# menickname/waafle

Hardware: AMD Instinct MI355X
Metric: contigs scored/sec + k2 clade-pair evals/sec at 1/2/4/8 MI355X vs CPU ref (higher is better)
Workload: dtype f64

## Files before the change

waafle_amd/csrc/wf_device.h:

```cpp
#pragma once
#include "wf_internal.h"

#include "waafle_hip.h"
#include "wf_lanes.h"

namespace wf {

namespace {


constexpr uint64_t kKeyPad = ~0ull;

#include "wf_stamps.h"
constexpr int kLocVirtual = 0xFFFF;

__device__ __forceinline__ void note_ppot(const KArgs& K, int c, int iteration, int Pp) {
  if (!K.ppot || Pp < 2) return;
  const uint64_t old = (uint64_t)K.ppot[c];
  if (iteration > (int)(old >> 40))
    K.ppot[c] = (int64_t)(((uint64_t)iteration << 40) | ((old & ((1ull << 40) - 1ull)) + (uint64_t)Pp));
}

__device__ __forceinline__ bool e2_no_option(const KArgs& K, int c, int iteration, int64_t pair_evals, bool root,
                                             int32_t* pend) {
// ... 309 lines not shown
    a7 = a6; a6 = a5; a5 = a4; a4 = a3; a3 = a2; a2 = a1; a1 = a0; a0 = v;
    pop();
    --sp;
    while (sp > 0) {
      if (ss[0] == 1) {
        int h = sl[0] / 2;
        h -= h % 8;
        ss[0] = 2;
        push(so[0] + h, sl[0] - h);
        ++sp;
        break;
      }
      a0 = a1 + a0;
      a1 = a2; a2 = a3; a3 = a4; a4 = a5; a5 = a6; a6 = a7;
      pop();
      --sp;
    }
  }
  return a0;
}

template <class F>
__device__ __forceinline__ double np_sum(int n, F f) {
  if (n <= kLeafMax) return 0.0 + serial_block(0, n, f);
  double total = 0.0;
  for (int o = 0; o < n; o += kNpyBuf) total += serial_pairwise(o, min(kNpyBuf, n - o), f);
  return total;
}


struct Contig {
  int64_t h0, l0, mbase;
  int H, G;
  int *loc_lo, *loc_len, *loc_st, *leaf_off;
  int *loc_grp, *loc_steps, *sched_off;
  uint64_t* sched;
  int4* leaves;
  int *alo, *ahi, *ahit, *aloc, *acl;
  double* asc;
  uint64_t* maxes;
  int *ign, *um;
  uint64_t* keys;
  int *seg_start, *seg_cl, *cl_id, *pot, *mem1, *mem2, *sorder;
  double* S;
  uint64_t* mask;
  unsigned *bm1, *bm2;
  uint8_t* best_syn;
  char* xws = nullptr;
  int64_t xcap = 0;
  int* sib_of = nullptr;
  uint64_t* hm = nullptr;
};

struct SumStack {
  double s0 = 0.0, s1 = 0.0, s2 = 0.0, s3 = 0.0, s4 = 0.0, s5 = 0.0, s6 = 0.0, s7 = 0.0;
  __device__ __forceinline__ void push(double v) {
    s7 = s6; s6 = s5; s5 = s4; s4 = s3; s3 = s2; s2 = s1; s1 = s0; s0 = v;
  }
  __device__ __forceinline__ void add_top() {
    s0 = s1 + s0;
    s1 = s2; s2 = s3; s3 = s4; s4 = s5; s5 = s6; s6 = s7;
  }
};

__device__ __forceinline__ double seqsum(double v, int cnt) {
  double r = 0.0;
  for (int i = 0; i < cnt; ++i) r += v;
  return r;
}

__device__ __forceinline__ double leaf_tree(double r0, double r1, double r2, double r3, double r4,
                                            double r5, double r6, double r7) {
  return ((r0 + r1) + (r2 + r3)) + ((r4 + r5) + (r6 + r7));
}

__device__ __forceinline__ int below(int base, int bound, int m) {
  const int d = bound - base;
  return d <= 0 ? 0 : min(m, (d + 7) >> 3);
}

constexpr int kThreadLeaves = 32;
constexpr int kE2Seg = 320;
constexpr int kE2MaxG = 63;
constexpr int kPruneMax = 64;

constexpr double kEnvSlack = 2e-12;
template <class Rg, class Sc>
__device__ __forceinline__ double env_integral(Rg range, Sc score, int kb, int ke, int len, double& best) {
  double acc = 0.0;
  best = 0.0;
  for (int p = 0; p < len;) {
    int nx = len;
    double val = 0.0;
    for (int q = kb; q < ke; ++q) {
      int l, h;
      range(q, l, h);
      if (l >= h) continue;
      if (l <= p && p < h) {
        const double s = score(q);
        val = s > val ? s : val;
        nx = h < nx ? h : nx;
      } else if (l > p) {
        nx = l < nx ? l : nx;
      }
    }
    best = val > best ? val : best;
    acc += val * (double)(nx - p);
    p = nx;
  }
  return acc / (double)len;
}
__device__ __forceinline__ double marker_ub(double v) { return -1.0 - v; }
__device__ __forceinline__ double marker_lb(double v) {
  const double ub = -1.0 - v;
  const double lb = ub * (1.0 - 5e-12) - 4.5e-16 * (1.0 + ub);
  return lb > 0.0 ? lb : 0.0;
}

__device__ __forceinline__ bool attaches(const DevParams& P, int qlo, int qhi, int hs, int l1,
                                         int len, int lst) {
  if (P.stranded && hs != lst) return false;
  const int l2 = l1 + len - 1;
  if (l1 > qhi || qlo > l2) return 0.0 >= P.min_overlap;
  const int ov = min(qhi, l2) - max(qlo, l1) + 1;
  const int den = min(qhi - qlo + 1, l2 - l1 + 1);
  if (ov == den) return 1.0 >= P.min_overlap;
  const double t = (double)den * P.min_overlap;
  if ((double)ov > t + fabs(t) * 1e-9) return true;
  if ((double)ov < t - fabs(t) * 1e-9) return false;
  return (double)ov / (double)den >= P.min_overlap;
}

__device__ __forceinline__ double run_leaf(int lo, int hi, double v, int st, int ln) {
  const int m = ln >> 3, be = st + (m << 3);
  hi = max(hi, lo);
  double res = 0.0;
  if (m > 0) {
    int k[8], kmin = m;
#pragma unroll
    for (int c = 0; c < 8; ++c) {
      k[c] = below(st + c, hi, m) - below(st + c, lo, m);
      kmin = min(kmin, k[c]);
    }
    double s0 = 0.0;
    for (int i = 0; i < kmin; ++i) s0 += v;
    const double s1 = s0 + v, s2 = s1 + v;
    double r[8];
#pragma unroll
    for (int c = 0; c < 8; ++c) r[c] = k[c] == kmin ? s0 : (k[c] == kmin + 1 ? s1 : s2);
    res = leaf_tree(r[0], r[1], r[2], r[3], r[4], r[5], r[6], r[7]);
  }
  for (int x = be; x < st + ln; ++x) res += (x >= lo && x < hi) ? v : 0.0;
  return res;
}

template <class F>
__device__ __forceinline__ double np_sum_seq(int n, F next) {
  if (n < 8) {
    double r = 0.0;
    for (int i = 0; i < n; ++i) r += next();
    return r;
  }
  double r0 = next(), r1 = next(), r2 = next(), r3 = next();
  double r4 = next(), r5 = next(), r6 = next(), r7 = next();
  int i = 8;
  const int m = n - (n & 7);
// ... 1339 lines not shown
```

waafle_amd/csrc/wf_sparse.h:

```cpp
constexpr int kSpCls = 128;
constexpr int kSpPairs = 128;
constexpr int kSpMemG = 2048;
constexpr int kSpParG = 4096;
constexpr int kSpDense = 16384;
constexpr int kSpWin = 256;
constexpr int kSpMaxG = 63;
constexpr int kSpP1 = 8;

struct SpMember {
  int rs, cl, pi, sp;
  int h, pad;
  unsigned long long hm;
};
struct SpParent {
  unsigned long long key, c1, c2, c3;
};
constexpr int kSpLPar = 64;
static_assert(kSpLPar * 32 == kSpCls * (8 + 4 + 4), "lpar overlays the class table");
constexpr int64_t kSpOffGidx = (int64_t)kSpMemG * sizeof(SpMember);
constexpr int64_t kSpOffPar = kSpOffGidx + (int64_t)kSpMemG * sizeof(int);
constexpr int64_t kSpOffDense = kSpOffPar + (int64_t)kSpParG * sizeof(SpParent);
constexpr int64_t kSpOffUrow = kSpOffDense + (int64_t)kSpDense * sizeof(double);
constexpr int64_t kSpOffBm = kSpOffUrow + 64 * sizeof(double);
constexpr int64_t kSpSlot = kSpOffBm + 2 * (kSpMemG / 32) * sizeof(unsigned);
// ... 800 lines not shown
      lca1 = a1;
      lca2v = a2;
      bool keepit = true;
      if (!P.allow_lca) {
        const int nl = lca2(K, lca1, lca2v);
        keepit = !(nl == lca1 || nl == lca2v);
      }
      have_ok = keepit;
    } else if (kind == 1) {
      have_ok = __shfl(best_ok, 0, 64) != 0;
    } else if (kind == 3) {
      have_ok = true;
    }
    if (have_ok) {
      if (lane < G) K.syn[l0 + lane] = sh.syn[lane];
      if (kind == 2) {
        int o1 = 0, o2 = 0;
        for (int base = 0; base < M; base += 64) {
          const int q = base + lane;
          const bool in1 = in_bm(bm1, q), in2 = in_bm(bm2, q);
          const uint64_t w1 = __ballot(in1), w2 = __ballot(in2);
          if (in1) K.meld[mbase + o1 + __popcll(w1 & below)] = mem[q].cl;
          if (in2) K.meld[mbase + m1 + o2 + __popcll(w2 & below)] = mem[q].cl;
          o1 += __popcll(w1);
          o2 += __popcll(w2);
        }
      }
      if (lane == 0) {
        K.call[c] = WF_CALL_LGT;
        K.crit[c] = best_crit;
        K.rank[c] = pr;
        K.dir[c] = (int8_t)best_dir;
        K.c1[c] = (kind == 2) ? lca1 : mem[best_c1].cl;
        K.c2[c] = (kind == 2) ? lca2v : mem[best_c2].cl;
        K.nm1[c] = (kind == 2) ? m1 : 0;
        K.nm2[c] = (kind == 2) ? m2 : 0;
        K.iters[c] = (int16_t)iteration;
        K.pair_evals[c] = pair_evals;
      }
      BLAP(9);
      return true;
    }
  }
  const int dec = (no_rows || root_present) ? kDecStop : kDecRaise;
  if (dec == kDecRaise && iteration + 1 <= kMaxIter) {
    if (S.seed_pend) {
      if (lane == 0) {
        S.seed_pend[c] = 2;
        K.pair_evals[c] = pair_evals;
      }
      return true;
    }
    sp_raise(S, c, pair_evals);
    BLAP(9);
    return true;
  }
  if (lane == 0) {
    const int it = dec == kDecRaise ? iteration + 1 : iteration;
    K.iters[c] = (int16_t)min(it, 32767);
    K.pair_evals[c] = pair_evals;
    K.status[c] = dec == kDecRaise ? WF_E_RUNAWAY : 0;
  }
  return true;
}

struct E2Shared {
  union {
    struct {
      int2 cg[kE2Seg];
      unsigned long long pm[64];
    };
    unsigned short cand[64 * 63 / 2];
  };
  double v[kE2Seg];
  int t[64], cl[64], par[64], sibp[64];
  unsigned long long pres[64], hm[64], s1[64], s2[64];
  int len[64];
};

__device__ __forceinline__ double e2_at(const E2Shared& sh, int t, uint64_t pres, int g) {
  return ((pres >> g) & 1ull) ? sh.v[t + __popcll(pres & ((1ull << g) - 1ull))] : 0.0;
}

__device__ __forceinline__ double e2_rank(const E2Shared& sh, int a, int b, uint64_t um, int Gu) {
  const int ta = sh.t[a], tb = sh.t[b];
  const uint64_t pa = sh.pres[a], pb = sh.pres[b];
  uint64_t m = um;
  auto next = [&]() -> double {
    const int g = __builtin_ctzll(m);
    m &= m - 1;
    const double x = e2_at(sh, ta, pa, g), y = e2_at(sh, tb, pb, g);
    return x < y ? y : x;
  };
  return (0.0 + np_sum_seq(Gu, next)) / (double)Gu;
}

struct E2Eval {
  int ok, swapped, dir;
  uint64_t mm, mA, mB;
};

__device__ __forceinline__ E2Eval e2_eval(const KArgs& K, const E2Shared& sh, int a, int b, uint64_t um) {
  const DevParams& P = K.p;
  const bool unk = sh.cl[a] == K.unknown || sh.cl[b] == K.unknown;
  uint64_t mm = 0, ma = 0, mb = 0;
  {
    const int ta = sh.t[a], tb = sh.t[b];
    const uint64_t pa = sh.pres[a], pb = sh.pres[b];
    for (uint64_t r = um; r; r &= r - 1) {
      const int g = __builtin_ctzll(r);
      const uint64_t bit = 1ull << g;
      const double s1 = e2_at(sh, ta, pa, g), s2 = e2_at(sh, tb, pb, g);
      const double mn = s2 < s1 ? s2 : s1;
      if (mn >= P.k_amb && !unk) mm |= bit;
      else if (s1 >= P.k2) ma |= bit;
      else if (s2 >= P.k2) mb |= bit;
    }
  }
  E2Eval e;
  const uint64_t ab = ma | mb;
  e.swapped = (ab && ((mb >> __builtin_ctzll(ab)) & 1ull)) ? 1 : 0;
  e.mm = mm;
  e.mA = e.swapped ? mb : ma;
  e.mB = e.swapped ? ma : mb;
  int64_t tot = 0, amb = 0;
  int state = 0;
  bool dir_ok = true;
  for (uint64_t r = um; r; r &= r - 1) {
    const int g = __builtin_ctzll(r);
    const uint64_t bit = 1ull << g;
    const char c = (mm & bit) ? '*' : (e.mA & bit) ? 'A' : (e.mB & bit) ? 'B' : '!';
    if (c != '!') {
      tot += sh.len[g];
      if (c == '*') amb += sh.len[g];
    }
    if (state == 0) { if (c == 'A') state = 1; else dir_ok = false; }
    else if (state == 1) { if (c == 'B') state = 2; else if (c != 'A') dir_ok = false; }
    else if (state == 2) { if (c == 'A') state = 3; else if (c != 'B') dir_ok = false; }
    else { if (c != 'A') dir_ok = false; }
  }
  e.dir = (dir_ok && state == 3) ? 1 : 0;
  e.ok = 1;
  if ((double)amb / (double)tot > P.amb_frac) e.ok = 0;
  if (P.clade_genes >= 0 && min(__popcll(e.mA), __popcll(e.mB)) < P.clade_genes) e.ok = 0;
  const int x = e.swapped ? b : a, y = e.swapped ? a : b;
  if (P.clade_leaves >= 0) {
    const int64_t ly = K.leaves[sh.cl[y]];
    const int64_t lc = e.dir ? ly : min(K.leaves[sh.cl[x]], ly);
    if (lc < P.clade_leaves) e.ok = 0;
  }
  if (P.sister_on && e.ok) {
    const int px = sh.par[x], py = sh.par[y];
    const uint64_t fb = sh.sibp[y] == px ? (sh.s2[x] | (sh.s1[x] & ~sh.hm[y])) : sh.s1[x];
    uint64_t fa = 0;
    if (!e.dir) fa = sh.sibp[x] == py ? (sh.s2[y] | (sh.s1[y] & ~sh.hm[x])) : sh.s1[y];
    if ((fb & e.mB) || (fa & e.mA)) e.ok = 0;
  }
  return e;
}

__device__ __forceinline__ int e2_wave_lca(const KArgs& K, int acc) {
#pragma unroll
  for (int off = 32; off > 0; off >>= 1) acc = lca2(K, acc, __shfl_xor(acc, off, 64));
  return acc;
}

__device__ __forceinline__ bool sp_two(const SArgs& S, E2Shared& sh, int c, int so, int se, uint64_t hdr,
                                       int64_t h0, int64_t l0, int G, int level) {
  const KArgs& K = S.k;
  const DevParams& P = K.p;
  const int lane = threadIdx.x & 63;
  const uint64_t below = (1ull << lane) - 1ull;
  const int ns = se - so;
  if (G > kE2MaxG || ns > kE2Seg) return false;
  SLAP_MARK(c);
  SSTAT(8, 1);
  SSTAT(9, ns);
  const uint64_t um = hdr & ~(1ull << 63);
  const bool root = (hdr >> 63) != 0ull;
  const int Gu = __popcll(um);
  const uint64_t allG = (1ull << G) - 1ull;
  const int iteration = level + 1;
  int64_t pair_evals = level == 0 ? 0 : K.pair_evals[c];
  constexpr int kCh = kE2Seg / 64;
  {
    int2 cgr[kCh];
    double vr[kCh];
#pragma unroll
    for (int k = 0; k < kCh; ++k) {
      const int q = 64 * k + lane;
      cgr[k] = make_int2(-1, 0);
      vr[k] = 0.0;
      if (q < ns) {
        cgr[k] = S.dump_cg[so + q];
        vr[k] = S.dump_mean[so + q];
      }
    }
    int ln = 0;
    if (lane < G) {
      const int ls = K.lstart[l0 + lane], le = K.lend[l0 + lane];
      ln = max(ls, le) - min(ls, le) + 1;
    }
#pragma unroll
    for (int k = 0; k < kCh; ++k) {
      const int q = 64 * k + lane;
      if (q < ns) {
        sh.cg[q] = cgr[k];
        sh.v[q] = vr[k];
      }
    }
    if (lane < G) sh.len[lane] = ln;
  }
  __syncthreads();
  SLAP(0);
  int Pp = 0;
  int hcl[kCh];
  uint64_t hh[kCh];
#pragma unroll
  for (int k = 0; k < kCh; ++k) {
    const int t = 64 * k + lane;
    bool pot = false;
    uint64_t pres = 0, mk2 = 0, hm = 0;
    int cl = -1;
    if (t < ns) {
      cl = sh.cg[t].x;
      if (t == 0 || sh.cg[t - 1].x != cl) {
        for (int q = t; q < ns && sh.cg[q].x == cl; ++q) {
          const uint64_t bit = 1ull << sh.cg[q].y;
          const double x = sh.v[q];
          pres |= bit;
          if (x >= P.k2) mk2 |= bit;
          if (x >= P.sister_thr) hm |= bit;
        }
        const uint64_t miss = allG & ~pres;
        if (0.0 >= P.k2) mk2 |= miss;
        if (0.0 >= P.sister_thr) hm |= miss;
        pot = mk2 != 0ull;
      } else {
        cl = -1;
      }
    }
    hcl[k] = cl;
    hh[k] = hm;
    const uint64_t pb = __ballot(pot);
    const int i = Pp + __popcll(pb & below);
    if (pot && i < 64) {
      sh.t[i] = t; sh.cl[i] = cl;
      sh.pres[i] = pres; sh.pm[i] = mk2 & um; sh.hm[i] = hm; sh.s1[i] = 0; sh.s2[i] = 0;
    }
    Pp += __popcll(pb);
  }
  if (Pp > 64) return false;
  __syncthreads();
  SLAP(1);
  SSTAT(10, Pp);
  const uint64_t my_pm = lane < Pp ? sh.pm[lane] : 0ull;
  pair_evals += (int64_t)Pp * (Pp - 1) / 2;
  if (lane == 0) note_ppot(K, c, iteration, Pp);
  __syncthreads();
  int nc = 0;
  const int n_pairs = Pp * (Pp - 1) / 2;
  for (int p0 = 0; p0 < n_pairs; p0 += 64) {
    const int p = min(p0 + lane, n_pairs - 1);
    int j = (int)((1.0f + __fsqrt_rn(1.0f + 8.0f * (float)p)) * 0.5f);
    j -= j * (j - 1) / 2 > p ? 1 : 0;
    j += (j + 1) * j / 2 <= p ? 1 : 0;
    const int i = p - j * (j - 1) / 2;
    const uint64_t mi = (uint64_t)__shfl((long long)my_pm, i, 64), mj = (uint64_t)__shfl((long long)my_pm, j, 64);
    const bool cand = p0 + lane < n_pairs && (mi | mj) == um;
    const uint64_t cb = __ballot(cand);
    if (cand) sh.cand[nc + __popcll(cb & below)] = (unsigned short)(i | (j << 8));
    nc += __popcll(cb);
  }
  __syncthreads();
  uint64_t memb = 0;
  for (int q = lane; q < nc; q += 64) memb |= (1ull << (sh.cand[q] & 0xFF)) | (1ull << (sh.cand[q] >> 8));
#pragma unroll
  for (int off = 32; off > 0; off >>= 1) memb |= (uint64_t)__shfl_xor((long long)memb, off, 64);
  SLAP(2);
  SSTAT(11, nc);
  if (P.sister_on && memb) {
    const bool me = (memb >> lane) & 1ull;
    const int my_cl = me ? sh.cl[lane] : -1;
    const int my_par = me ? K.parent[my_cl] : -2;
    if (me) {
      sh.par[lane] = my_par;
      sh.sibp[lane] = K.sibp[my_cl];
    }
    int hsp[kCh];
#pragma unroll
    for (int k = 0; k < kCh; ++k) hsp[k] = (hcl[k] >= 0 && hh[k] != 0ull) ? K.sibp[hcl[k]] : -1;
    uint64_t s1 = 0, s2 = 0;
#pragma unroll
    for (int k = 0; k < kCh; ++k) {
      if (64 * k >= ns) break;
      const int sp = hsp[k], cl = hcl[k];
      const uint64_t h = hh[k];
      bool match = false;
      for (uint64_t r = memb; r; r &= r - 1) match = match || (sp >= 0 && sp == lane_bcast(my_par, __builtin_ctzll(r)));
      for (uint64_t mb = __ballot(match); mb; mb &= mb - 1) {
        const int src = __builtin_ctzll(mb);
        const int sp_r = lane_bcast(sp, src), cl_r = lane_bcast(cl, src);
        const uint64_t h_r = lane_bcast(h, src);
        if (my_par == sp_r && my_cl != cl_r) {
          s2 |= s1 & h_r;
          s1 |= h_r;
        }
      }
    }
    if (me) { sh.s1[lane] = s1; sh.s2[lane] = s2; }
    __syncthreads();
  }
  SLAP(3);
  double pr = -__builtin_inf();
  long long pk = -1;
  if (nc > 0) {
    for (int q = lane; q < nc; q += 64) {
      const int i = sh.cand[q] & 0xFF, j = sh.cand[q] >> 8;
      const double r = e2_rank(sh, i, j, um, Gu);
      const long long key = (long long)i * Pp + j;
      if (better(r, key, pr, pk)) { pr = r; pk = key; }
    }
    each_stride([&](auto J) {
      constexpr int js = decltype(J)::value;
      const double r2 = xor_lanes<js>(pr);
      const long long k2 = xor_lanes<js>(pk);
      if (better(r2, k2, pr, pk)) { pr = r2; pk = k2; }
    });
  }
  SLAP(4);
  if (pk >= 0) {
    const int bi = (int)(pk / Pp), bj = (int)(pk % Pp);
    const E2Eval be = e2_eval(K, sh, bi, bj, um);
    int n_in = 0;
    bool all_ok = true, all_same = true;
    uint64_t b1 = 0, b2 = 0;
    for (int q = lane; q < nc; q += 64) {
      const int i = sh.cand[q] & 0xFF, j = sh.cand[q] >> 8;
      if ((pr - e2_rank(sh, i, j, um, Gu)) <= P.range) {
        const E2Eval e = e2_eval(K, sh, i, j, um);
        ++n_in;
        all_ok = all_ok && e.ok;
        all_same = all_same && e.mm == be.mm && e.mA == be.mA && e.mB == be.mB;
        b1 |= 1ull << (e.swapped ? j : i);
        b2 |= 1ull << (e.swapped ? i : j);
      }
    }
#pragma unroll
    for (int off = 32; off > 0; off >>= 1) {
      n_in += __shfl_xor(n_in, off, 64);
      b1 |= (uint64_t)__shfl_xor((long long)b1, off, 64);
      b2 |= (uint64_t)__shfl_xor((long long)b2, off, 64);
    }
    all_ok = __ballot(!all_ok) == 0ull;
    all_same = __ballot(!all_same) == 0ull;
    int kind;
    if (n_in == 0) kind = (P.dis2 == 0) ? 3 : (P.dis2 == 1 ? 0 : 4);
    else if (n_in == 1 || P.dis2 == 0) kind = 1;
    else if (P.dis2 == 1) kind = 0;
    else kind = (all_ok && all_same) ? 2 : 0;
    if (kind == 4) {
      if (lane == 0) K.status[c] = WF_E_BADINPUT;
      return true;
    }
    bool have_ok = false;
    int lca1 = -1, lca2v = -1;
    const bool in1 = (b1 >> lane) & 1ull, in2 = (b2 >> lane) & 1ull;
    const int my_cl = lane < Pp ? sh.cl[lane] : -1;
    if (kind == 2) {
      lca1 = e2_wave_lca(K, in1 ? my_cl : -1);
      lca2v = e2_wave_lca(K, in2 ? my_cl : -1);
      bool keep = true;
      if (!P.allow_lca) {
        const int nl = lca2(K, lca1, lca2v);
        keep = !(nl == lca1 || nl == lca2v);
      }
      have_ok = keep;
    } else if (kind == 1) {
      have_ok = be.ok != 0;
    } else if (kind == 3) {
      have_ok = true;
    }
    if (have_ok) {
      const int64_t mbase = 2 * h0 + 2 * (int64_t)c;
      const int m1 = __popcll(b1), m2 = __popcll(b2);
      if (kind == 2) {
        if (in1) K.meld[mbase + __popcll(b1 & below)] = my_cl;
        if (in2) K.meld[mbase + m1 + __popcll(b2 & below)] = my_cl;
      }
      if (lane < G) {
        const uint64_t bit = 1ull << lane;
        K.syn[l0 + lane] = !(um & bit) ? '~' : (be.mm & bit) ? '*' : (be.mA & bit) ? 'A' : (be.mB & bit) ? 'B' : '!';
      }
      if (lane == 0) {
        double bcrit = 0.0;
        bool first = true;
        const int ta = sh.t[bi], tb = sh.t[bj];
        const uint64_t pa = sh.pres[bi], pb = sh.pres[bj];
        for (uint64_t r = um; r; r &= r - 1) {
          const int g = __builtin_ctzll(r);
          const double x = e2_at(sh, ta, pa, g), y = e2_at(sh, tb, pb, g);
          const double m = x < y ? y : x;
          bcrit = (first || m < bcrit) ? m : bcrit;
          first = false;
        }
        K.call[c] = WF_CALL_LGT;
        K.crit[c] = bcrit;
        K.rank[c] = pr;
        K.dir[c] = (int8_t)be.dir;
        K.c1[c] = kind == 2 ? lca1 : sh.cl[be.swapped ? bj : bi];
        K.c2[c] = kind == 2 ? lca2v : sh.cl[be.swapped ? bi : bj];
        K.nm1[c] = kind == 2 ? m1 : 0;
        K.nm2[c] = kind == 2 ? m2 : 0;
        K.iters[c] = (int16_t)iteration;
        K.pair_evals[c] = pair_evals;
      }
      SLAP(5);
      return true;
    }
  }
  SLAP(5);
  e2_no_option(K, c, iteration, pair_evals, root, S.seed_pend);
  return true;
}

__global__ __launch_bounds__(64, 4) void k_big_sparse(const SArgs S_arg, int level, int64_t n_keys) {
  __shared__ SpShared sh;
  char* ws = S_arg.sp_ws + (int64_t)blockIdx.x * kSpSlot;
  const int count = (int)S_arg.counters[2];
  for (int i = blockIdx.x; i < count; i += gridDim.x) {
    const SArgs& S = kernarg_fresh<SArgs>(S_arg);
    const int cr = S.big_list[2 * i], c = S.big_list[2 * i + 1];
    const bool ok = sp_level(S, sh, ws, c, cr, level, n_keys);
    if (!ok && threadIdx.x == 0) {
      const int slot = (int)atomicAdd(&S.counters[1], 1ull);
      S.big2_list[2 * slot] = cr;
      S.big2_list[2 * slot + 1] = c;
    }
    __syncthreads();
  }
}

template <int KIND>
__global__ __launch_bounds__(64, KIND ? 4 : 2) void k_dump_sparse(const SArgs S_arg, int64_t* ccnt, int64_t* cleaves,
                                                                  int level) {
  using Sh = typename std::conditional<KIND == 1, E2Shared, SpShared>::type;
  __shared__ Sh sh;
  const int lane = threadIdx.x & 63;
  const SArgs& S0 = S_arg;
  if (KIND == 1) {
    if (S0.dump_ctr_next && blockIdx.x == 0 && lane == 0) *S0.dump_ctr_next = 0ull;
    if (S0.anc) {
      const int up = level == 0 ? S0.k.p.jump + 1 : 1;
      for (int t = blockIdx.x * 64 + lane; t < S0.n_tax; t += gridDim.x * 64) {
        int x = level == 0 ? t : S0.anc[t];
        for (int j = 0; j < up; ++j) x = S0.k.parent[x];
        S0.anc[t] = x;
      }
    }
  }
  char* ws = KIND ? nullptr : S0.sp_ws + (int64_t)blockIdx.x * kSpSlot;
  const int count = (int)(*S0.dump_ctr >> 40);
  const int stride = (int)gridDim.x;
  auto finish = [&](const SArgs& S, int c, bool ok) {
    if (lane == 0) {
      const int pd = S.seed_pend[c];
      if (!ok) {
        S.seed_pend[c] = 1;
        if (S.fail_ctr) atomicAdd(S.fail_ctr, 1ull);
      } else if (pd == 3) {
        S.seed_pend[c] = 0;
        ccnt[c] = 0;
        cleaves[c] = 0;
      } else if (pd == 2 && S.roll_next) {
        S.roll_next[atomicAdd(S.roll_next_n, 1ull)] = c;
      }
    }
    __syncthreads();
  };
  for (int base = blockIdx.x; base < count; base += 64 * stride) {
    const int my = base + lane * stride;
    int mc = -1, so = 0, se = 0, G = 0;
    uint64_t hdr = 0;
    int64_t h0 = 0, l0 = 0;
    if (my < count) {
      const int2 dl = reinterpret_cast<const int2*>(S0.dump_list)[my];
      if (dl.x == KIND && dl.y >= 0) {
        mc = dl.y;
        if (KIND == 1) {
          so = S0.dump_first[my];
// ... 25 lines not shown
```

waafle_amd/csrc/wf_staged.hip:

```cpp
#include <hipcub/hipcub.hpp>

#include <algorithm>
#include <atomic>
#include <cstdlib>
#include <string>
#include <vector>

#include "wf_attach.h"

namespace wf {

namespace {

__device__ __forceinline__ int upper_index(const int64_t* off, int n, int64_t x) {
  int lo = 0, hi = n - 1;
  while (lo < hi) {
    const int mid = (lo + hi + 1) >> 1;
    if (off[mid] <= x) lo = mid; else hi = mid - 1;
  }
  return lo;
}

__device__ __forceinline__ int lower_bound_i32(const int32_t* a, int n, int x) {
  int lo = 0, hi = n;
// ... 1438 lines not shown
        cl[r] = a < a1 ? S.att_clade[a] : 0;
      }
#pragma unroll
      for (int r = 0; r < 4; ++r) cl[r] = K.parent[cl[r]];
#pragma unroll
      for (int r = 0; r < 4; ++r) {
        const int64_t a = ab + r * NT + tid;
        if (a < a1) S.att_clade[a] = cl[r];
      }
    }
    STAMP_SYNC();
    STAMP(19);
    return true;
  }
  if (tid == 0) {
    const int it = dec == kDecRaise ? iteration + 1 : iteration;
    K.iters[c] = (int16_t)min(it, 32767);
    K.pair_evals[c] = pair_evals;
    K.status[c] = dec == kDecRaise ? WF_E_RUNAWAY : ctl.status;
  }
  return true;
}

constexpr int kDecNT = 64;

template <int PHASE, int NT = kDecNT>
__global__ __launch_bounds__(NT, 2) void k_decide(const SArgs S, int n_act,
                                                   int level, int64_t n_keys) {
  lvl_counts(S, n_act, n_keys);
  extern __shared__ __attribute__((aligned(16))) char smem[];
  __shared__ Ctl ctl;
  if constexpr (PHASE == 3) {
    const int c1 = (int)S.counters[6], c2 = (int)S.counters[5];
    for (int i = blockIdx.x; i < c1 + c2; i += gridDim.x) {
      const bool whole = i < c1;
      const int32_t* L = whole ? S.one_list : S.two_list;
      const int j = whole ? i : i - c1;
      const int cr = L[2 * j], c = L[2 * j + 1];
      const bool ok = whole ? decide_contig<NT, 0>(S, c, cr, level, smem, S.dec_lds_bytes, ctl, n_keys)
                            : decide_contig<NT, 2>(S, c, cr, level, smem, S.dec_lds_bytes, ctl, n_keys);
      if (!ok && threadIdx.x == 0) {
        const int slot = (int)atomicAdd(&S.counters[2], 1ull);
        S.big_list[2 * slot] = cr;
        S.big_list[2 * slot + 1] = c;
        atomicMax(&S.counters[3], (unsigned long long)S.k.need[c]);
      }
      __syncthreads();
    }
  } else {
  const int32_t* list = PHASE == 1 ? S.one_list : S.two_list;
  const int count = PHASE == 1 ? (list ? (int)S.counters[6] : n_act) : (int)S.counters[5];
  for (int i = blockIdx.x; i < count; i += gridDim.x) {
    const int cr = list ? list[2 * i] : i;
    const int c = list ? list[2 * i + 1] : (S.act ? S.act[cr] : cr);
    const bool ok = decide_contig<NT, PHASE>(S, c, cr, level, smem, S.dec_lds_bytes, ctl, n_keys);
    if (!ok && threadIdx.x == 0) {
      const int slot = (int)atomicAdd(&S.counters[2], 1ull);
      S.big_list[2 * slot] = cr;
      S.big_list[2 * slot + 1] = c;
      atomicMax(&S.counters[3], (unsigned long long)S.k.need[c]);
    }
    __syncthreads();
  }
  }
}

__global__ __launch_bounds__(kBlock, 2) void k_decide_big(const SArgs S, int level,
                                                          int64_t n_keys, int use2) {
  int n_act_ = 0;
  lvl_counts(S, n_act_, n_keys);
  const int count = (int)S.counters[use2 ? 1 : 2];
  const int32_t* list = use2 ? S.big2_list : S.big_list;
  __shared__ Ctl ctl;
  char* base = S.k.big_ws + (int64_t)blockIdx.x * S.k.slot_bytes;
  for (int i = blockIdx.x; i < count; i += gridDim.x) {
    const int cr = list[2 * i], c = list[2 * i + 1];
    const bool ok = decide_contig<kBlock, 0>(S, c, cr, level, base, S.k.slot_bytes, ctl, n_keys, false);
    if (!ok && threadIdx.x == 0) S.k.status[c] = WF_E_NOMEM;
    __syncthreads();
  }
}

#include "wf_sparse.h"
WF_STAMP_READER(sparse, g_sstamps, 16)
WF_STAMP_READER(big, g_bstamps, 48)

int bits_for(int64_t v) {
  int b = 1;
  while (b < 62 && (int64_t(1) << b) <= v) ++b;
  return b;
}

struct Buf {
  void* p = nullptr;
  size_t n = 0;
  ~Buf() { if (p) (void)hipFree(p); }
  hipError_t ensure(hipStream_t drain, size_t bytes) {
    if (bytes <= n) return hipSuccess;
    if (p) {
      hipError_t e = hipStreamSynchronize(drain);
      if (e != hipSuccess) return e;
      (void)hipFree(p);
      p = nullptr;
      n = 0;
    }
    size_t want = std::max<size_t>(bytes + bytes / 4, 256);
    hipError_t e = hipMalloc(&p, want);
    if (e == hipSuccess) n = want;
    return e;
  }
  template <class T> T* as() const { return static_cast<T*>(p); }
};

}



struct StagedState {
  int device = 0;
  int cus = 256;
  Buf lut_off, lut, cnt, att_off, counters, pinned_dummy;
  Buf att_lo, att_hi, att_loc, att_clade, att_hit, att_sc;
  Buf keys0, keys1, vals0, vals1, flags, seg_id, seg_start, seg_crank, seg_mean;
  Buf cnt_leaves, red, seg_nleaf, leaf_off, leaf_seg, leaf_val, annot_best;
  Buf seg_rec, seg_cg, crank_first, satt_lohi, satt_sc, wave_list, lvl_ctr, seg_cnt, seg_len;
  Buf front;
  Buf span_cnt, spans;
  unsigned long long* host_lvl = nullptr;
  hipEvent_t lvl_ev[2] = {nullptr, nullptr};
  int sparse_big = 3;
  int sparse_res = -1;
  int two_res = -1;
  int64_t att_limit = (int64_t(1) << 31) - 1;
  int64_t dump_cap = 0;
  int triage = 1;
  int wave_two = 2;
  Buf tri_list, tri_cnt;
  Buf wq;
  Buf roll0, roll1, roll_cnt, anc;
  bool timing = false;
  std::vector<hipEvent_t> tev;
  int tev_used = 0;
  std::vector<int> tspans;
  double phase_ms[8] = {0};
  int64_t phase_n[8] = {0};
  Buf act0, act1, base0, base1, big_list, big2_list, two_list, one_list, big_ws, tmp, pend, act_l0;
  Buf sp_ws;
  Buf hkey;
  Buf dump_cg, dump_mean, dump_first, dump_list, dump_ctr, dump_um;
  bool level0 = true;
  bool rollup = false;
  bool lut_ready = false;
  int64_t dec_lds = 32 * 1024;
  bool dec_lds_fixed = false;
  unsigned long long* host_counters = nullptr;
  unsigned long long* mbox = nullptr;
  unsigned long long* mbox_dev = nullptr;
  unsigned long long mbox_seq = 0;
  ~StagedState() {
    for (hipEvent_t e : tev) (void)hipEventDestroy(e);
    if (mbox) (void)hipHostFree(mbox);
    if (host_counters) (void)hipHostFree(host_counters);
    if (host_lvl) (void)hipHostFree(host_lvl);
    for (hipEvent_t e : lvl_ev)
      if (e) (void)hipEventDestroy(e);
  }
};
// ... 863 lines not shown
```

waafle_amd/csrc/wf_stamps.h:

```cpp
#pragma once
#ifdef WF_STAMPS
#ifndef WF_STAMPS_ROLL
#define WF_STAMPS_ROLL 0
#endif
#define WF_STAMPS_ONLY(...) __VA_ARGS__
#define WF_STAMP_READER(tag, arr, n)                                                          \
  extern "C" int wf_stamps_read_##tag(unsigned long long* out, int m) {                       \
    if (m > (n)) m = (n);                                                                     \
    return hipMemcpyFromSymbol(out, HIP_SYMBOL(arr), sizeof(unsigned long long) * m) == hipSuccess ? 0 : -2; \
  }                                                                                           \
  extern "C" int wf_stamps_reset_##tag(void) {                                                \
    unsigned long long z[n] = {0};                                                            \
    return hipMemcpyToSymbol(HIP_SYMBOL(arr), z, sizeof z) == hipSuccess ? 0 : -2;            \
  }
__device__ unsigned long long g_stamps[32];
__shared__ unsigned long long g_tlast;
#define STAMP_INIT() do { if (threadIdx.x == 0) g_tlast = __builtin_amdgcn_s_memtime(); } while (0)
#define STAMP(i)                                                                    \
  do {                                                                              \
    if (threadIdx.x == 0) {                                                         \
      unsigned long long now_ = __builtin_amdgcn_s_memtime();                       \
      atomicAdd(&g_stamps[i], now_ - g_tlast);                                      \
      g_tlast = now_;                                                               \
    }                                                                               \
  } while (0)
#define STAMP_SYNC() __syncthreads()
#define LAP_MARK() unsigned long long lap_ = __builtin_amdgcn_s_memtime()
#define LAP(i)                                                                      \
  do {                                                                              \
    unsigned long long n_ = __builtin_amdgcn_s_memtime();                           \
    if (threadIdx.x == 0) atomicAdd(&g_stamps[i], n_ - lap_);                       \
    lap_ = n_;                                                                      \
  } while (0)
#define LAP_WAIT_LDS() __builtin_amdgcn_s_waitcnt(0xc07f)
#define LAP_WAIT_V(v) asm volatile("" ::"v"(v))
#define STAT(i, v) do { if (threadIdx.x == 0) atomicAdd(&g_stamps[i], (unsigned long long)(v)); } while (0)
__device__ unsigned long long g_wstamps[48];
#define WLAP_MARK() unsigned long long wlap_ = __builtin_amdgcn_s_memtime(); const bool wsamp_ = !FULL && (WF_STAMPS_ROLL ? ROLL : !ROLL) && (c & 15) == 0
#define WLAP(i)                                                                     \
  do {                                                                              \
    const unsigned long long n_ = __builtin_amdgcn_s_memtime();                     \
    if (wsamp_ && lane == 0) atomicAdd(&g_wstamps[i], n_ - wlap_);                  \
    wlap_ = n_;                                                                     \
  } while (0)
#define WSTAT(i, v) do { if (wsamp_ && lane == 0) atomicAdd(&g_wstamps[i], (unsigned long long)(v)); } while (0)
__device__ unsigned long long g_tstamps[16];
#define TLAP_MARK() unsigned long long tlap_ = __builtin_amdgcn_s_memtime(); const bool tsamp_ = (c & 15) == 0
#define TLAP(i)                                                                     \
  do {                                                                              \
    const unsigned long long n_ = __builtin_amdgcn_s_memtime();                     \
    if (tsamp_ && lane == 0) atomicAdd(&g_tstamps[i], n_ - tlap_);                  \
    tlap_ = n_;                                                                     \
  } while (0)
__device__ unsigned long long g_sstamps[16];
#define SLAP_MARK(c) unsigned long long slap_ = __builtin_amdgcn_s_memtime(); const bool ssamp_ = ((c) & 7) == 0
#define SLAP(i)                                                                     \
  do {                                                                              \
    const unsigned long long n_ = __builtin_amdgcn_s_memtime();                     \
    if (ssamp_ && (threadIdx.x & 63) == 0) atomicAdd(&g_sstamps[i], n_ - slap_);    \
    slap_ = n_;                                                                     \
  } while (0)
#define SSTAT(i, v) do { if (ssamp_ && (threadIdx.x & 63) == 0) atomicAdd(&g_sstamps[i], (unsigned long long)(v)); } while (0)
__device__ unsigned long long g_bstamps[48];
#define BLAP_MARK(c) unsigned long long blap_ = __builtin_amdgcn_s_memtime(); const bool bsamp_ = ((c) & 7) == 0
#define BLAP(i)                                                                     \
  do {                                                                              \
    const unsigned long long n_ = __builtin_amdgcn_s_memtime();                     \
    if (bsamp_ && (threadIdx.x & 63) == 0) {                                        \
      atomicAdd(&g_bstamps[i], n_ - blap_);                                         \
      if (level > 0) atomicAdd(&g_bstamps[24 + (i)], n_ - blap_);                   \
    }                                                                               \
    blap_ = n_;                                                                     \
  } while (0)
#define BSTAT(i, v) do { if (bsamp_ && (threadIdx.x & 63) == 0) atomicAdd(&g_bstamps[i], (unsigned long long)(v)); } while (0)
#else
#define WF_STAMPS_ONLY(...)
#define WF_STAMP_READER(tag, arr, n)
#define STAMP_INIT() do {} while (0)
#define STAMP(i) do {} while (0)
#define STAMP_SYNC() do {} while (0)
#define LAP_MARK() do {} while (0)
#define LAP(i) do {} while (0)
#define LAP_WAIT_LDS() do {} while (0)
#define LAP_WAIT_V(v) do {} while (0)
#define STAT(i, v) do {} while (0)
#define WLAP_MARK() do {} while (0)
#define WLAP(i) do {} while (0)
#define WSTAT(i, v) do {} while (0)
#define TLAP_MARK() do {} while (0)
#define TLAP(i) do {} while (0)
#define BLAP_MARK(c) do {} while (0)
#define BLAP(i) do {} while (0)
#define BSTAT(i, v) do {} while (0)
#define SLAP_MARK(c) do {} while (0)
#define SLAP(i) do {} while (0)
#define SSTAT(i, v) do {} while (0)
#endif
```

Before: 116.5 million.

## Evaluate few E2 candidate pairs wave-cooperatively and cache per-pair evaluations

Merges rank, crit and classification into a single per-pair evaluation, so each candidate's gene scores are read once instead of separately for rank, best-pair eval, in-range eval and crit. When there are at most eight candidates, each pair is evaluated across the 64 lanes using ballots and DPP reductions instead of one lane doing a serial loop. The direction state machine becomes bitmask arithmetic, and the cross-lane reductions switch to DPP helpers. In exchange it adds register pressure from carrying a full E2Eval per lane, and it widens the stamp counters.

```diff
diff --git a/waafle_amd/csrc/wf_device.h b/waafle_amd/csrc/wf_device.h
--- a/waafle_amd/csrc/wf_device.h
+++ b/waafle_amd/csrc/wf_device.h
@@ -415,6 +415,10 @@
 constexpr int kThreadLeaves = 32;
 constexpr int kE2Seg = 320;
 constexpr int kE2MaxG = 63;
+#ifndef WF_E2_WAVE_PAIRS
+#define WF_E2_WAVE_PAIRS 8
+#endif
+constexpr int kE2WavePairs = WF_E2_WAVE_PAIRS;
 constexpr int kPruneMax = 64;
 
 constexpr double kEnvSlack = 2e-12;
diff --git a/waafle_amd/csrc/wf_sparse.h b/waafle_amd/csrc/wf_sparse.h
--- a/waafle_amd/csrc/wf_sparse.h
+++ b/waafle_amd/csrc/wf_sparse.h
@@ -906,64 +906,27 @@
   return ((pres >> g) & 1ull) ? sh.v[t + __popcll(pres & ((1ull << g) - 1ull))] : 0.0;
 }
 
-__device__ __forceinline__ double e2_rank(const E2Shared& sh, int a, int b, uint64_t um, int Gu) {
-  const int ta = sh.t[a], tb = sh.t[b];
-  const uint64_t pa = sh.pres[a], pb = sh.pres[b];
-  uint64_t m = um;
-  auto next = [&]() -> double {
-    const int g = __builtin_ctzll(m);
-    m &= m - 1;
-    const double x = e2_at(sh, ta, pa, g), y = e2_at(sh, tb, pb, g);
-    return x < y ? y : x;
-  };
-  return (0.0 + np_sum_seq(Gu, next)) / (double)Gu;
-}
-
 struct E2Eval {
-  int ok, swapped, dir;
+  double rank, crit;
+  unsigned ok : 1, swapped : 1, dir : 1;
   uint64_t mm, mA, mB;
 };
 
-__device__ __forceinline__ E2Eval e2_eval(const KArgs& K, const E2Shared& sh, int a, int b, uint64_t um) {
+__device__ __forceinline__ void e2_checks(const KArgs& K, const E2Shared& sh, int a, int b, uint64_t um,
+                                          uint64_t mm, uint64_t ma, uint64_t mb, int64_t tot, int64_t amb,
+                                          E2Eval& e) {
   const DevParams& P = K.p;
-  const bool unk = sh.cl[a] == K.unknown || sh.cl[b] == K.unknown;
-  uint64_t mm = 0, ma = 0, mb = 0;
-  {
-    const int ta = sh.t[a], tb = sh.t[b];
-    const uint64_t pa = sh.pres[a], pb = sh.pres[b];
-    for (uint64_t r = um; r; r &= r - 1) {
-      const int g = __builtin_ctzll(r);
-      const uint64_t bit = 1ull << g;
-      const double s1 = e2_at(sh, ta, pa, g), s2 = e2_at(sh, tb, pb, g);
-      const double mn = s2 < s1 ? s2 : s1;
-      if (mn >= P.k_amb && !unk) mm |= bit;
-      else if (s1 >= P.k2) ma |= bit;
-      else if (s2 >= P.k2) mb |= bit;
-    }
-  }
-  E2Eval e;
   const uint64_t ab = ma | mb;
   e.swapped = (ab && ((mb >> __builtin_ctzll(ab)) & 1ull)) ? 1 : 0;
   e.mm = mm;
   e.mA = e.swapped ? mb : ma;
   e.mB = e.swapped ? ma : mb;
-  int64_t tot = 0, amb = 0;
-  int state = 0;
-  bool dir_ok = true;
-  for (uint64_t r = um; r; r &= r - 1) {
-    const int g = __builtin_ctzll(r);
-    const uint64_t bit = 1ull << g;
-    const char c = (mm & bit) ? '*' : (e.mA & bit) ? 'A' : (e.mB & bit) ? 'B' : '!';
-    if (c != '!') {
-      tot += sh.len[g];
-      if (c == '*') amb += sh.len[g];
-    }
-    if (state == 0) { if (c == 'A') state = 1; else dir_ok = false; }
-    else if (state == 1) { if (c == 'B') state = 2; else if (c != 'A') dir_ok = false; }
-    else if (state == 2) { if (c == 'A') state = 3; else if (c != 'B') dir_ok = false; }
-    else { if (c != 'A') dir_ok = false; }
-  }
-  e.dir = (dir_ok && state == 3) ? 1 : 0;
+  e.dir = 0;
+  if (e.mB && (e.mA | e.mB) == um) {
+    const int lo = __builtin_ctzll(e.mB), hi = 63 - __builtin_clzll(e.mB);
+    const uint64_t from_lo = ~0ull << lo, to_hi = ~0ull >> (63 - hi);
+    e.dir = ((from_lo & to_hi & um) == e.mB && (e.mA & ~from_lo) && (e.mA & ~to_hi)) ? 1 : 0;
+  }
   e.ok = 1;
   if ((double)amb / (double)tot > P.amb_frac) e.ok = 0;
   if (P.clade_genes >= 0 && min(__popcll(e.mA), __popcll(e.mB)) < P.clade_genes) e.ok = 0;
@@ -980,7 +943,82 @@
     if (!e.dir) fa = sh.sibp[x] == py ? (sh.s2[y] | (sh.s1[y] & ~sh.hm[x])) : sh.s1[y];
     if ((fb & e.mB) || (fa & e.mA)) e.ok = 0;
   }
+}
+
+__device__ __forceinline__ E2Eval e2_pair(const KArgs& K, const E2Shared& sh, int a, int b, uint64_t um, int Gu) {
+  const DevParams& P = K.p;
+  const bool unk = sh.cl[a] == K.unknown || sh.cl[b] == K.unknown;
+  const int ta = sh.t[a], tb = sh.t[b];
+  const uint64_t pa = sh.pres[a], pb = sh.pres[b];
+  E2Eval e;
+  uint64_t m = um;
+  auto next = [&]() -> double {
+    const int g = __builtin_ctzll(m);
+    m &= m - 1;
+    const double x = e2_at(sh, ta, pa, g), y = e2_at(sh, tb, pb, g);
+    return x < y ? y : x;
+  };
+  e.rank = (0.0 + np_sum_seq(Gu, next)) / (double)Gu;
+  uint64_t mm = 0, ma = 0, mb = 0;
+  int64_t tot = 0, amb = 0;
+  double crit = 0.0;
+  for (uint64_t r = um; r; r &= r - 1) {
+    const int g = __builtin_ctzll(r);
+    const uint64_t bit = 1ull << g;
+    const double s1 = e2_at(sh, ta, pa, g), s2 = e2_at(sh, tb, pb, g);
+    const double mn = s2 < s1 ? s2 : s1, mx = s1 < s2 ? s2 : s1;
+    crit = (r == um || mx < crit) ? mx : crit;
+    if (mn >= P.k_amb && !unk) mm |= bit;
+    else if (s1 >= P.k2) ma |= bit;
+    else if (s2 >= P.k2) mb |= bit;
+    else continue;
+    tot += sh.len[g];
+    if (mm & bit) amb += sh.len[g];
+  }
+  e.crit = crit;
+  e2_checks(K, sh, a, b, um, mm, ma, mb, tot, amb, e);
   return e;
+}
+
+__device__ __forceinline__ E2Eval e2_pair_wave(const KArgs& K, const E2Shared& sh, int a, int b, uint64_t um, int Gu) {
+  const DevParams& P = K.p;
+  const int lane = threadIdx.x & 63;
+  const bool in = (um >> lane) & 1ull;
+  const int ln = in ? sh.len[lane] : 0;
+  const bool unk = sh.cl[a] == K.unknown || sh.cl[b] == K.unknown;
+  const double s1 = e2_at(sh, sh.t[a], sh.pres[a], lane), s2 = e2_at(sh, sh.t[b], sh.pres[b], lane);
+  const double mn = s2 < s1 ? s2 : s1, mx = s1 < s2 ? s2 : s1;
+  E2Eval e;
+  uint64_t m = um;
+  auto next = [&]() -> double {
+    const int g = __builtin_ctzll(m);
+    m &= m - 1;
+    return lane_bcast(mx, g);
+  };
+  e.rank = (0.0 + np_sum_seq(Gu, next)) / (double)Gu;
+  const double lo = wave_butterfly(in ? mx : __builtin_inf(), [](double p, double q) { return q < p ? q : p; });
+  e.crit = Gu ? lo : 0.0;
+  const bool star = in && mn >= P.k_amb && !unk;
+  const bool isa = in && !star && s1 >= P.k2;
+  const bool isb = in && !star && !isa && s2 >= P.k2;
+  const uint64_t mm = __ballot(star), ma = __ballot(isa), mb = __ballot(isb);
+  const int64_t tot = wave_sum_dpp((long long)((star || isa || isb) ? ln : 0));
+  const int64_t amb = mm ? wave_sum_dpp((long long)(star ? ln : 0)) : 0;
+  e2_checks(K, sh, a, b, um, mm, ma, mb, tot, amb, e);
+  return e;
+}
+
+__device__ __forceinline__ E2Eval e2_bcast(const E2Eval& e, int src) {
+  E2Eval r;
+  r.rank = lane_bcast(e.rank, src);
+  r.crit = lane_bcast(e.crit, src);
+  r.ok = lane_bcast((int)e.ok, src);
+  r.swapped = lane_bcast((int)e.swapped, src);
+  r.dir = lane_bcast((int)e.dir, src);
+  r.mm = lane_bcast(e.mm, src);
+  r.mA = lane_bcast(e.mA, src);
+  r.mB = lane_bcast(e.mB, src);
+  return r;
 }
 
 __device__ __forceinline__ int e2_wave_lca(const KArgs& K, int acc) {
@@ -1099,10 +1137,10 @@
   __syncthreads();
   uint64_t memb = 0;
   for (int q = lane; q < nc; q += 64) memb |= (1ull << (sh.cand[q] & 0xFF)) | (1ull << (sh.cand[q] >> 8));
-#pragma unroll
-  for (int off = 32; off > 0; off >>= 1) memb |= (uint64_t)__shfl_xor((long long)memb, off, 64);
+  memb = wave_or_dpp(memb);
   SLAP(2);
   SSTAT(11, nc);
+  SSTAT(nc == 0 ? 25 : 15 + min(nc, 9), 1);
   if (P.sister_on && memb) {
     const bool me = (memb >> lane) & 1ull;
     const int my_cl = me ? sh.cl[lane] : -1;
@@ -1137,32 +1175,43 @@
   }
   SLAP(3);
   double pr = -__builtin_inf();
-  long long pk = -1;
-  if (nc > 0) {
+  int pk = -1, bi = 0, bj = 0;
+  E2Eval mine = {}, be = {};
+  if (nc > 0 && nc <= kE2WavePairs) {
+    SSTAT(26, 1);
+    for (int q = 0; q < nc; ++q) {
+      const int i = sh.cand[q] & 0xFF, j = sh.cand[q] >> 8;
+      const E2Eval e = e2_pair_wave(K, sh, i, j, um, Gu);
+      if (lane == q) mine = e;
+      if (better(e.rank, i * Pp + j, pr, pk)) { pr = e.rank; pk = i * Pp + j; bi = i; bj = j; be = e; }
+    }
+  } else if (nc > 0) {
     for (int q = lane; q < nc; q += 64) {
       const int i = sh.cand[q] & 0xFF, j = sh.cand[q] >> 8;
-      const double r = e2_rank(sh, i, j, um, Gu);
-      const long long key = (long long)i * Pp + j;
-      if (better(r, key, pr, pk)) { pr = r; pk = key; }
+      const E2Eval e = e2_pair(K, sh, i, j, um, Gu);
+      if (q < 64) mine = e;
+      if (better(e.rank, i * Pp + j, pr, pk)) { pr = e.rank; pk = i * Pp + j; }
     }
     each_stride([&](auto J) {
       constexpr int js = decltype(J)::value;
       const double r2 = xor_lanes<js>(pr);
-      const long long k2 = xor_lanes<js>(pk);
+      const int k2 = xor_lanes<js>(pk);
       if (better(r2, k2, pr, pk)) { pr = r2; pk = k2; }
     });
+    bi = pk / Pp, bj = pk % Pp;
+    const bool mine_best = lane < nc && sh.cand[lane] == (bi | (bj << 8));
+    be = nc <= 64 ? e2_bcast(mine, __builtin_ctzll(__ballot(mine_best))) : e2_pair(K, sh, bi, bj, um, Gu);
   }
   SLAP(4);
   if (pk >= 0) {
-    const int bi = (int)(pk / Pp), bj = (int)(pk % Pp);
-    const E2Eval be = e2_eval(K, sh, bi, bj, um);
     int n_in = 0;
     bool all_ok = true, all_same = true;
     uint64_t b1 = 0, b2 = 0;
     for (int q = lane; q < nc; q += 64) {
       const int i = sh.cand[q] & 0xFF, j = sh.cand[q] >> 8;
-      if ((pr - e2_rank(sh, i, j, um, Gu)) <= P.range) {
-        const E2Eval e = e2_eval(K, sh, i, j, um);
+      E2Eval e = mine;
+      if (q >= 64) e = e2_pair(K, sh, i, j, um, Gu);
+      if ((pr - e.rank) <= P.range) {
         ++n_in;
         all_ok = all_ok && e.ok;
         all_same = all_same && e.mm == be.mm && e.mA == be.mA && e.mB == be.mB;
@@ -1170,12 +1219,9 @@
         b2 |= 1ull << (e.swapped ? i : j);
       }
     }
-#pragma unroll
-    for (int off = 32; off > 0; off >>= 1) {
-      n_in += __shfl_xor(n_in, off, 64);
-      b1 |= (uint64_t)__shfl_xor((long long)b1, off, 64);
-      b2 |= (uint64_t)__shfl_xor((long long)b2, off, 64);
-    }
+    n_in = wave_sum_dpp(n_in);
+    b1 = wave_or_dpp(b1);
+    b2 = wave_or_dpp(b2);
     all_ok = __ballot(!all_ok) == 0ull;
     all_same = __ballot(!all_same) == 0ull;
     int kind;
@@ -1217,19 +1263,8 @@
         K.syn[l0 + lane] = !(um & bit) ? '~' : (be.mm & bit) ? '*' : (be.mA & bit) ? 'A' : (be.mB & bit) ? 'B' : '!';
       }
       if (lane == 0) {
-        double bcrit = 0.0;
-        bool first = true;
-        const int ta = sh.t[bi], tb = sh.t[bj];
-        const uint64_t pa = sh.pres[bi], pb = sh.pres[bj];
-        for (uint64_t r = um; r; r &= r - 1) {
-          const int g = __builtin_ctzll(r);
-          const double x = e2_at(sh, ta, pa, g), y = e2_at(sh, tb, pb, g);
-          const double m = x < y ? y : x;
-          bcrit = (first || m < bcrit) ? m : bcrit;
-          first = false;
-        }
         K.call[c] = WF_CALL_LGT;
-        K.crit[c] = bcrit;
+        K.crit[c] = be.crit;
         K.rank[c] = pr;
         K.dir[c] = (int8_t)be.dir;
         K.c1[c] = kind == 2 ? lca1 : sh.cl[be.swapped ? bj : bi];
diff --git a/waafle_amd/csrc/wf_staged.hip b/waafle_amd/csrc/wf_staged.hip
--- a/waafle_amd/csrc/wf_staged.hip
+++ b/waafle_amd/csrc/wf_staged.hip
@@ -1544,7 +1544,7 @@
 }
 
 #include "wf_sparse.h"
-WF_STAMP_READER(sparse, g_sstamps, 16)
+WF_STAMP_READER(sparse, g_sstamps, 32)
 WF_STAMP_READER(big, g_bstamps, 48)
 
 int bits_for(int64_t v) {
diff --git a/waafle_amd/csrc/wf_stamps.h b/waafle_amd/csrc/wf_stamps.h
--- a/waafle_amd/csrc/wf_stamps.h
+++ b/waafle_amd/csrc/wf_stamps.h
@@ -52,7 +52,7 @@
     if (tsamp_ && lane == 0) atomicAdd(&g_tstamps[i], n_ - tlap_);                  \
     tlap_ = n_;                                                                     \
   } while (0)
-__device__ unsigned long long g_sstamps[16];
+__device__ unsigned long long g_sstamps[32];
 #define SLAP_MARK(c) unsigned long long slap_ = __builtin_amdgcn_s_memtime(); const bool ssamp_ = ((c) & 7) == 0
 #define SLAP(i)                                                                     \
   do {                                                                              \
```

After: 123.2 million, median of 6. 1.06x the previous value.
